# opteroncx/MoePhoto

Measured on AMD Instinct MI355X. Metric: megapixels/sec (input), 1080p 4x SR (Net4x a4), 256-px tiles with overlap, higher is better.
Workload: dtype fp16; 1 GPU; BASELINE configs[1]: 1 frame(s) 1920x1080 RGB -> 7680x4320, model a4 (Net4x, synthetic weights in zoo format), crop 256 pad 5 align 8 -> 40 tiles/frame, fp16 I/O, fp16 MFMA operands + fp32 accumulate; tiles_per_frame=40, parallelism=single GPU, precision=mixed, exact_blocks=1, input=natural-image-like synthetic frame (tests/golden_defs.natural_image)

## Files before the change

moephoto_amd/csrc/common.h:

```cpp
#pragma once
#include <hip/hip_runtime.h>
#include <stdint.h>

typedef _Float16 half_t;
typedef __attribute__((ext_vector_type(2))) _Float16 half2_t;
typedef __attribute__((ext_vector_type(4))) _Float16 half4_t;
typedef __attribute__((ext_vector_type(8))) _Float16 half8_t;
typedef __attribute__((ext_vector_type(4))) float float4_t;
typedef __attribute__((ext_vector_type(16))) float float16_t;

constexpr int kCB = 64;
constexpr int kTileW = 32;
constexpr int kTileH = 8;
constexpr int kFragBytes = 1024;

struct ConvArgs {
    const half_t* in;
    half_t* out;
    const half_t* res;
    const half_t* wpk;
    const float* bias;
    const float* bias_img;
    const half_t* zero;
    half_t* trash;
// ... 103 lines not shown
    const half_t* tail_w;
    half_t* out;
    float* plane;
    float* apron;
    float slope;
    int B, H, W;
    int split;
};
bool launch_conv3x3_ps4(const Ps4Args& a, int max_groups, hipStream_t s);
bool ps4_applicable(int B, int H, int W);
inline bool ps4_tail_applicable(int B, int H, int W, float slope) { return slope < 1.f && ps4_applicable(B, H, W); }
bool ps4_store_applicable(int B, int H, int W, float slope);
size_t ps4_plane_bytes(int B, int H, int W);
size_t ps4_apron_bytes(int B, int H, int W);
hipError_t conv3x3_ps4_init();
struct TailAddArgs {
    const float* p0; const float* p1;
    const float* a0; const float* a1;
    void* y; int y_dtype; const long long* y_off;
    int B, H, W, px;
    int vec_ok;
};
void launch_tailadd(const TailAddArgs& a, hipStream_t s);

struct Ps9Args {
    const half_t* in;
    const half_t* wpk;
    const float* bias;
    const half_t* tail_w;
    float* plane;
    float* apron;
    float slope;
    int B, H, W;
    int split;
    int xcd_map;
};
// ... 198 lines not shown
};
void launch_frm_pre(const FrmPreArgs& a, hipStream_t s);

struct StitchArgs {
    const float* tiles; const long long* tile_off;
    const int* row_first; const int* row_cnt;
    const int* col_first; const int* col_cnt;
    const int* row_tab; const int* col_tab;
    const float* ramp;
    void* out; int out_dtype;
    int C, out_h, out_w, step_w;
    int row_lo;
    int y0, rows;
};
void launch_stitch(const StitchArgs& a, hipStream_t s);

struct BlendTileArgs {
    const void* r; void* canvas; const void* ramp;
    long long r_sC, r_sH, c_sC, c_sH;
    int C, rh, rw;
    int top_sc, left_sc;
    int r0, c0;
    int lt_h, lt_w;
};
void launch_blend_tile(const BlendTileArgs& a, bool f16, hipStream_t s);

struct WireRec {
    long long tile_off, wire_off;
    int C, th, tw;
    int ra0, ra1, rb0, rb1;
// ... 12 lines not shown
```

moephoto_amd/csrc/conv3x3_ps4.hip:

```cpp
#include "common.h"
#include "rowtile.h"
#include "../../include/moephoto_amd.h"
#include <algorithm>
#include <type_traits>

#ifndef PS4_FILL
#define PS4_FILL 5
#endif
#ifndef PS4_ZSKIP
#define PS4_ZSKIP 1
#endif
#ifndef PS4_ABL
#define PS4_ABL 0
#endif

namespace {

constexpr int RB = 4;
constexpr int PW = kTileW + 2;
constexpr int ROWB = PW * 128;
constexpr int BLKB = RB * ROWB;
constexpr int NPIECE = BLKB / 1024;
constexpr int TREC = 36 * 128 + 64;
constexpr int TEXP = 36 * 128;
// ... 456 lines not shown
        typedef std::integral_constant<int, 0> Run;
        typedef std::integral_constant<int, 1> Zero;
        typedef std::integral_constant<int, 2> Last;
        int k = kfirst;
        for (; k + 1 < kz; k += 2) {
            block(k, std::integral_constant<int, 0>{}, Run{});
            block(k + 1, std::integral_constant<int, 1>{}, Run{});
        }
        if (k < kz) { block(k, std::integral_constant<int, 0>{}, Run{}); ++k; }
        if (k < nblk - 1) { block(k, std::integral_constant<int, 0>{}, Zero{}); ++k; }
        if (TAIL) block(k, std::integral_constant<int, 0>{}, Last{});
    }
#endif
}

template <bool VEC>
__global__ __launch_bounds__(256) void tailadd_kernel(TailAddArgs a)
{
    const int nq = a.W >> 3;
    const long long idx = (long long)blockIdx.x * 256 + threadIdx.x;
    if (idx >= (long long)a.B * a.H * nq) return;
    const int xq = (int)(idx % nq);
    const int Y = (int)((idx / nq) % a.H), b = (int)(idx / ((long long)nq * a.H));
    const int X0 = xq * 8;
    const long long po = ((long long)b * a.H + Y) * a.W + X0;
    float v[8];
    {
        const float4 r0 = *(const float4*)(a.p0 + po), r1 = *(const float4*)(a.p0 + po + 4);
        v[0] = r0.x; v[1] = r0.y; v[2] = r0.z; v[3] = r0.w; v[4] = r1.x; v[5] = r1.y; v[6] = r1.z; v[7] = r1.w;
        if (a.p1) {
            const float4 u0 = *(const float4*)(a.p1 + po), u1 = *(const float4*)(a.p1 + po + 4);
            v[0] += u0.x; v[1] += u0.y; v[2] += u0.z; v[3] += u0.w; v[4] += u1.x; v[5] += u1.y; v[6] += u1.z; v[7] += u1.w;
        }
    }
    const int c = X0 >> 6, in = X0 & 63;
    const long long as = (long long)a.B * a.px * a.H;
    if (in == 0 && c >= 1) {
        const long long o = ((long long)b * a.px + (c - 1)) * a.H + Y;
        float t = a.a0[o];
        if (a.a1) t += a.a1[o];
        v[0] += t;
    }
    if (in == 56 && c + 1 < a.px) {
        const long long o = as + ((long long)b * a.px + (c + 1)) * a.H + Y;
        float t = a.a0[o];
        if (a.a1) t += a.a1[o];
        v[7] += t;
    }
    const long long yo = (a.y_off ? a.y_off[b] : (long long)b * a.H * a.W) + (long long)Y * a.W + X0;
    if (a.y_dtype == MOE_F16) {
        if (VEC) {
            half8_t h;
#pragma unroll
            for (int k = 0; k < 8; ++k) h[k] = (half_t)v[k];
            *(half8_t*)((half_t*)a.y + yo) = h;
        } else {
#pragma unroll
            for (int k = 0; k < 8; ++k) ((half_t*)a.y)[yo + k] = (half_t)v[k];
        }
    } else {
        float* yp = (float*)a.y + yo;
        if (VEC) {
            *(float4*)yp = make_float4(v[0], v[1], v[2], v[3]);
            *(float4*)(yp + 4) = make_float4(v[4], v[5], v[6], v[7]);
        } else {
#pragma unroll
            for (int k = 0; k < 8; ++k) yp[k] = v[k];
        }
    }
}

template <int EPI, bool MASK>
hipError_t set_limit()
{
    return hipFuncSetAttribute((const void*)conv3x3_ps4_kernel<EPI, MASK>, hipFuncAttributeMaxDynamicSharedMemorySize, LDS_BYTES);
}

}

hipError_t conv3x3_ps4_init()
{
    hipError_t e;
    if ((e = set_limit<0, true>()) != hipSuccess) return e;
    if ((e = set_limit<1, false>()) != hipSuccess) return e;
// ... 49 lines not shown
```

moephoto_amd/csrc/engine.h:

```cpp
#pragma once
#include <cstdint>
#include <map>
#include <memory>
#include <string>
#include <utility>
#include <vector>

#include "../../include/moephoto_amd.h"
#include "common.h"

namespace moe {

struct AxisAnchors {
    std::vector<int64_t> start, end, end_sc;
    int64_t clip = 0;
    int step = 1;
};
AxisAnchors get_anchors(int64_t s, int64_t ns, int64_t l, int pad, int align, int sc);

struct TileRect { int top, bottom, left, right, top_t, left_t, bsc, rsc; };

struct PlanDeviceCache {
    int device = -1;
    int C = 0;
    int64_t sC = 0, sH = 0, sW = 0;
    int shard_index = 0, shard_count = 1;
    bool y_mult8 = false;
    std::vector<int> group_first, group_count;
    void* blob = nullptr;
    long long* x_off = nullptr;
    long long* y_off = nullptr;
    long long* tile_off = nullptr;
    int *row_first = nullptr, *row_cnt = nullptr, *col_first = nullptr, *col_cnt = nullptr, *row_tab = nullptr, *col_tab = nullptr;
    float* ramp = nullptr;
    std::vector<std::pair<int, int*>> strip_tabs;
};

struct FramesDeviceCache {
    int device = -1, C = 0, n_frames = 0;
    int64_t sC = 0, sH = 0, sW = 0, frame_stride = 0;
    std::vector<long long> tile_dst;
    bool y_mult8 = false;
    std::vector<int> group_first, group_count;
    void* blob = nullptr;
    long long* x_off = nullptr;
    long long* y_off = nullptr;
};

struct CustomOffsets { int device; std::vector<long long> host; long long* dev; };
// ... 24 lines not shown
```

moephoto_amd/csrc/forward.cpp:

```cpp
#include "net.h"

using namespace moe;

namespace moe {

const char* kernel_name(ConvKernel k)
{
    static const char* const names[] = {"no kernel", "conv_direct", "conv1x1", "conv_mfma", "conv3x3_sp", "conv3x3_rw", "conv3x3_ps4 (store form)", "conv3x3_sp (hi + lo residual)",
                                        "conv_mfma (three products)", "conv64_x3", "conv64_q8", "conv64_sq", "conv3x3_sp (three launches)", "conv_mfma (fp32 side buffer)"};
    return names[(int)k];
}

static bool fast_layer(const moe_net& n, const ConvLayer& L) { return L.taps == 9 && L.nseg == 1 && !L.per_plane && n.opt.conv_impl == 2; }

ConvForm Fwd::form(const ConvLayer& L, int H, int W) const
{
    ConvForm c;
    c.B = B; c.H = H; c.W = W; c.in_cs = 64 * L.nseg; c.out_cs = L.r > 1 ? 64 : 64 * L.nchunks; c.r = L.r; c.nchunks = L.nchunks;
    c.py = (H + kTileH - 1) / kTileH;
    const long long items = (long long)B * ((W + kTileW - 1) / kTileW) * c.py;
    const int per_xcd = groups / 8;
    int G = per_xcd >= L.nchunks ? 8 * (per_xcd / L.nchunks) : groups / L.nchunks;
    if (G < 1) G = 1;
    if (G > items) G = (int)items;
// ... 371 lines not shown
    if ((io.x_dtype != MOE_F32 && io.x_dtype != MOE_F16) || (io.y_dtype != MOE_F32 && io.y_dtype != MOE_F16))
        return fail(MOE_EINVAL, "moe_net_forward: x/y dtype must be MOE_F32 or MOE_F16");
    const long long bmax = kSpRange / (sp_bytes_per_pixel(n) * (long long)h * w);
    if (bmax < 1)
        return fail(MOE_ENOMEM, "a %dx%d tile exceeds the convolution kernels' addressing range (%lld pixels per plane at most for this net): use a smaller cropsize",
                    h, w, kSpRange / sp_bytes_per_pixel(n));
    if (n.arch == MOE_ARCH_LITE && io.x_dtype == MOE_F16 && n.lut_state == 0 && n.opt.lite_lut) build_lite_lut(n, s, ctx);
    if (B <= bmax) return forward_dev_chunk(n, io, B, h, w, s, y_off_mult8, ctx);
    const size_t xe = io.x_dtype == MOE_F32 ? 4 : 2, ye = io.y_dtype == MOE_F32 ? 4 : 2;
    const long long yplane = (long long)h * n.scale * w * n.scale;
    for (int b0 = 0; b0 < B; b0 += (int)bmax) {
        const int cnt = (int)std::min<long long>(bmax, B - b0);
        FwdIO c = io;
        if (io.x_off) c.x_off += b0; else c.x = (const char*)io.x + (size_t)b0 * io.sB * xe;
        if (io.y_off) c.y_off += b0; else c.y = (char*)io.y + (size_t)b0 * yplane * ye;
        const bool al = y_off_mult8 && (io.y_off || ((size_t)b0 * yplane * ye) % 16 == 0);
        if (int rc = forward_dev_chunk(n, c, cnt, h, w, s, al, ctx)) return rc;
    }
    return MOE_OK;
}

static int forward_dev_chunk(moe_net& n, const FwdIO& io, int B, int h, int w, hipStream_t s, bool y_off_mult8, const FwdCtx& ctx)
{
    int cur = -1;
    HIP_TRY(hipGetDevice(&cur));
    if (cur != n.device) HIP_TRY(hipSetDevice(n.device));
    const size_t need = workspace_need(n, ctx, B, h, w);
    StreamSet& set = *ctx.set;
    if (need > set.ws_bytes) {
        if (set.ws) { HIP_TRY(hipStreamSynchronize(s)); HIP_TRY(hipFree(set.ws)); set.ws = nullptr; set.ws_bytes = 0; }
        hipError_t e = hipMalloc((void**)&set.ws, need);
        if (e != hipSuccess) { (void)hipGetLastError(); return fail(MOE_ENOMEM, "workspace of %zu bytes for %d planes of %dx%d does not fit", need, B, h, w); }
        set.ws_bytes = need;
    }
// ... 210 lines not shown
```

moephoto_amd/csrc/forward_arsb.cpp:

```cpp
#include "net.h"

using namespace moe;

namespace {

const ConvLayer* last_up(const moe_net& n, int br)
{
    const auto it = n.conv_index.find(std::string(br == 0 ? "convt_R1" : "u") + ".up" + std::to_string(n.stages - 1));
    return it == n.conv_index.end() ? nullptr : &n.convs[it->second];
}

bool can_fuse_tail(const moe_net& n, const Fwd& f)
{
    const int B = f.B, h = f.h, w = f.w;
    if (!n.opt.fuse_tail || f.x3 || f.direct || n.debug || n.opt.conv_impl != 2 || n.stages < 1) return false;
    if (!(n.arch == MOE_ARCH_NET2X || n.arch == MOE_ARCH_NET3X || n.arch == MOE_ARCH_NET4X)) return false;
    if (sp_bytes_per_pixel(n) * B * h * w > kSpRange) return false;
    int hl = h, wl = w;
    for (int st = 0; st + 1 < n.stages; ++st) { hl *= n.r; wl *= n.r; }
    for (int br = 0; br < 2; ++br) {
        const ConvLayer* L = last_up(n, br);
        if (!L) return false;
        ConvForm c = f.form(*L, hl, wl);
        c.tail = true;
// ... 39 lines not shown
        bool ok = fuse && n.opt.tail_form == 1;
        bool ps4_ok = true;
        bool ps9_ok = true;
        for (int br = 0; br < 2; ++br) {
            const ConvLayer* L = last_up(n, br);
            if (ok) {
                ConvForm c = f.form(*L, hl, wl);
                c.tail = true; c.tail_form = 1;
                ok = conv3x3_rw_applicable(c);
            }
            ps4_ok = ps4_ok && L && ps4_tail_applicable(B, hl, wl, L->slope);
            ps9_ok = ps9_ok && L && ps9_tail_applicable(B, hl, wl, L->slope);
        }
        f.tail_form = ok ? 1 : 0;
        ps4 = ok && n.opt.up_impl == 1 && ps4_ok && (2 * wl) % 8 == 0;
        ps9 = fuse && n.opt.up_impl == 1 && n.r == 3 && f.groups >= 3 && ps9_ok;
    }
}

template <typename Args, typename Launch>
int ArsbRun::ps_stage(int br, const std::string& key, const Act& cur, size_t plane_bytes, size_t apron_bytes, const char* name, Launch launch)
{
    ps_plane[br] = (float*)f.ar.take(plane_bytes + 4096);
    ps_apron[br] = (float*)f.ar.take(apron_bytes + 4096);
    if (!f.dry()) {
        const ConvLayer& L = n.convs[n.conv_index.at(key)];
        Args q{};
        q.in = cur.hi; q.wpk = f.blob<half_t>(L.w_hi); q.bias = L.has_bias ? f.blob<float>(L.bias) : f.small<float>("zero_bias");
        q.tail_w = f.small<half_t>(br == 0 ? "tail_r.frag" : "tail_u.frag");
        q.plane = ps_plane[br]; q.apron = ps_apron[br]; q.slope = L.slope; q.B = B; q.H = H; q.W = W;
// ... 120 lines not shown
        if (int rc = trunk_conv(k2, m, cur, &resid, ex)) return rc;
        f.tap("arsb" + std::to_string(i), cur, h, w, 64, n.C);
    }
    Bb = cur;
    return (int)MOE_OK;
}

template <typename Args, typename Launch>
void ArsbRun::tail_add(Launch launch)
{
    if (f.dry()) return;
    Args t{};
    t.p0 = ps_plane[0]; t.p1 = ps_plane[1]; t.a0 = ps_apron[0]; t.a1 = ps_apron[1];
    t.y = f.io.y; t.y_dtype = f.io.y_dtype; t.y_off = f.io.y_off; t.B = B; t.H = H; t.W = W; t.px = (W / n.r + kTileW - 1) / kTileW;
    t.vec_ok = f.y_vec;
    const int rec = f.prof_begin("tailadd", 0.0);
    f.gate();
    launch(t, f.s);
    f.prof_end(rec);
}

int ArsbRun::branch_sum()
{
    if (ps4) { tail_add<TailAddArgs>(launch_tailadd); return MOE_OK; }
    if (ps9) { tail_add<TailAdd3Args>(launch_tailadd3); return MOE_OK; }
    if (fuse) {
        if (!f.dry()) {
            TapSumArgs t{};
            t.t0 = tp[0]; t.t1 = tp[1]; t.y = f.io.y; t.y_dtype = f.io.y_dtype; t.y_off = f.io.y_off; t.B = B; t.H = H; t.W = W; t.r = n.r;
            t.form = f.tail_form;
            t.vec_ok = n.r == 2 && f.y_vec && W % 8 == 0;
            f.gate();
            launch_tapsum(t, f.s);
        }
        return MOE_OK;
    }
    f.tail(&fin[0], &fin[1], H, W, false);
    return MOE_OK;
// ... 79 lines not shown
```

moephoto_amd/csrc/misc_kernels.hip:

```cpp
#include "common.h"
#include <algorithm>
#include <cstdlib>
#include <cstring>
#include "../../include/moephoto_amd.h"

namespace {

__device__ __forceinline__ float prelu(float v, float slope) { return v >= 0.f ? v : v * slope; }

template <typename T>
__device__ __forceinline__ float ld1(const void* p, long long i) { return (float)((const T*)p)[i]; }

template <typename TIN, int TAPS>
__global__ __launch_bounds__(256) void stem_kernel(StemArgs a)
{
    __shared__ float w[TAPS * 64];
    for (int i = threadIdx.x; i < TAPS * 64; i += 256) w[i] = a.w[i];
    __syncthreads();
    if (a.out_lo8) asm volatile("s_setreg_imm32_b32 hwreg(HW_REG_MODE, 23, 1), 1\n\ts_nop 3" ::: "memory");
    constexpr int PX = 8;
    const int nq = (a.W + PX - 1) / PX;
    const long long idx = (long long)blockIdx.x * 256 + threadIdx.x;
    const long long q = idx >> 3;
    if (q >= (long long)a.B * a.H * nq) return;
// ... 1091 lines not shown
    }
    __syncthreads();
    const int total = s_nseam * 8 * R;
    for (int t = threadIdx.x; t < total; t += 256) {
        const int gidx = t / (8 * R), rem = t - gidx * 8 * R;
        const int r = rem >> 3, e = rem & 7;
        const int X = (blockIdx.x * 256 + s_seam[gidx]) * 8 + e, Y = Y0 + r;
        if (Y >= yend) continue;
        const float cur = stitch_pixel(a, X, Y, c);
        const long long o = ((long long)c * a.rows + (Y - a.y0)) * a.out_w + X;
        if (a.out_dtype == MOE_F16) ((half_t*)a.out)[o] = (half_t)cur;
        else ((float*)a.out)[o] = cur;
    }
}

template <typename TS, typename TD>
__global__ void to_float_kernel(const TS* src, TD* dst, int H, int W, int C, float d, bool divide)
{
    const long long idx = (long long)blockIdx.x * 256 + threadIdx.x;
    const long long n = (long long)H * W * C;
    if (idx >= n) return;
    const int c = (int)(idx % C);
    const long long p = idx / C;
    const float v = (float)src[idx];
    dst[(long long)c * H * W + p] = (TD)(divide ? v / d : v * d);
}

template <typename TS, typename TD>
__global__ void to_output_kernel(const TS* src, TD* dst, int H, int W, int C, float quant)
{
// ... 143 lines not shown
    const long long total = (long long)a.B * a.HW * 8;
    hipLaunchKernelGGL(frm_apply_kernel, dim3((unsigned)((total + 255) / 256)), dim3(256), 0, s, a);
}

void launch_frm_pre(const FrmPreArgs& a, hipStream_t s)
{
    hipLaunchKernelGGL(frm_pre_kernel, dim3(a.B), dim3(256), 0, s, a);
}

void launch_stitch(const StitchArgs& a, hipStream_t s)
{
    if (a.rows <= 0) return;
    if (a.out_w % 8 == 0 && a.step_w <= 64 && ((uintptr_t)a.out & 15) == 0) hipLaunchKernelGGL(stitch8r_kernel<4>, dim3((a.out_w / 8 + 255) / 256, (a.rows + 3) / 4, a.C), dim3(256), 0, s, a);
    else if (a.out_w % 4 == 0 && ((uintptr_t)a.out & 15) == 0) hipLaunchKernelGGL(stitch4_kernel, dim3((a.out_w / 4 + 255) / 256, a.rows, a.C), dim3(256), 0, s, a);
    else hipLaunchKernelGGL(stitch_kernel, dim3((a.out_w + 255) / 256, a.rows, a.C), dim3(256), 0, s, a);
}

__device__ __forceinline__ int wire_slot(int v, int a0, int a1, int b0, int b1)
{
    return (v >= a0 && v < a1) ? v - a0 : (v >= b0 && v < b1) ? (a1 - a0) + v - b0 : -1;
}

template <bool PACK>
__global__ __launch_bounds__(256) void wire_kernel(float* __restrict__ tiles, unsigned* __restrict__ wire, const WireRec* __restrict__ recs)
{
    const WireRec r = recs[blockIdx.y];
    const int nR = (r.ra1 - r.ra0) + (r.rb1 - r.rb0), nC = (r.ca1 - r.ca0) + (r.cb1 - r.cb0);
    const bool raw = nR >= r.th;
    const long long plane = (long long)r.th * r.tw, n = plane * r.C;
    float* t = tiles + r.tile_off;
// ... 185 lines not shown
```

moephoto_amd/csrc/net.h:

```cpp
#pragma once
#include "engine.h"

#include <algorithm>
#include <cmath>
#include <cstdarg>
#include <cstdio>
#include <cstdlib>
#include <cstring>

namespace moe {

int fail(int code, const char* fmt, ...);

#define HIP_TRY(expr)                                                                                    \
    do {                                                                                                 \
        hipError_t e_ = (expr);                                                                          \
        if (e_ != hipSuccess) return fail(e_ == hipErrorOutOfMemory ? MOE_ENOMEM : MOE_EHIP, "%s: %s", #expr, hipGetErrorString(e_)); \
    } while (0)

struct Param {
    std::string name;
    std::vector<int64_t> shape;
    std::vector<float> data;
    bool set = false;
// ... 49 lines not shown
    int k48 = 1;
    int s64 = 1;
    int branch_streams = 1;
    int branch_groups = 0;
    int exact_fuse = 1;
    int q8_impl = 1;
    int fuse_tail = 1;
    int sedn_fuse = 1;
    int pool_fuse = 1;
    int lite_lut = 1;
    int stem2 = 1;
    int frm_pre = 1;
    int overlap_calls = 1;
    int overlap_fork = 0;
    int overlap_groups = 0;
    int calib_log = 0;
    int auto_calibrate = 1;
    int exact_blocks_env = -1;
    int tiles_per_batch = 0;
    int max_groups = 0;
    int dbg = 0;
    std::string trace_key = "convt_R1.up1";
    bool arsb_trace = false;
    std::string repeat_key;
    int repeat_n = 1;


    bool set(const std::string& key, const char* v);
    void from_env();
};
// ... 51 lines not shown
        return it == index.end() ? nullptr : &params[it->second];
    }
    void add(const std::string& n, std::vector<int64_t> shape)
    {
        index[n] = (int)params.size();
        moe::Param p; p.name = n; p.shape = std::move(shape);
        params.push_back(std::move(p));
    }
};

namespace moe {

struct FwdIO {
    const void* x = nullptr; int x_dtype = MOE_F32; long long sB = 0, sH = 0, sW = 0; const long long* x_off = nullptr;
    void* y = nullptr; int y_dtype = MOE_F32; const long long* y_off = nullptr;
};

struct FwdCtx {
    StreamSet* set = nullptr;
    int groups = 0;
    bool fork = false;
    hipEvent_t gate_event = nullptr;
    float* lut_capture = nullptr;
};
inline FwdCtx own_ctx(const moe_net& n, StreamSet* set) { return FwdCtx{set, n.max_groups, n.opt.branch_streams != 0, nullptr, nullptr}; }

struct ConvExtra {
    const half_t* plane_w = nullptr;
    const half_t* plane_w_lo = nullptr;
    const half_t* tail_w = nullptr;
// ... 17 lines not shown
enum class ConvKernel {
    none, direct, conv1x1,
    mfma, sp, rw, ps4_store,
    sp_res_lo,
    mfma_x3,
    x3, q8, sq,
    sp_three, acc32,
};
struct ConvRoute {
    ConvKernel kernel = ConvKernel::none;
    ConvDone done;
    ConvForm form;
    ConvX3Form x3;
};
const char* kernel_name(ConvKernel k);

struct Fwd {
    const moe_net& n;
    const FwdCtx& ctx;
    NetRuntime* rt;
    hipStream_t s;
    int B, h, w;
    Arena ar;
    int groups;
    bool x3, direct;
    bool mixed = false;
    bool y_vec = false;
    float* acc32 = nullptr;
    size_t acc32_elems = 0;
    half_t* side16 = nullptr;
    bool dry() const { return ar.base == nullptr; }
    int rc = 0;
    bool skips_planned_work = false;
    int tail_form = 0;
    FwdIO io;

    Act act(long long pixels, int ch = 64, bool want_lo = false)
    {
        Act a;
        a.hi = (half_t*)ar.take((size_t)pixels * ch * 2 + 2048);
        if (x3 || want_lo) { a.lo = (half_t*)ar.take((size_t)pixels * ch * 2 + 2048); a.has_lo = true; }
        return a;
    }
    template <typename T> T* blob(size_t off) const { return (T*)(n.blob + off); }
    template <typename T> T* small(const std::string& k) const { return (T*)(n.blob + n.small.at(k)); }

    void tap(const std::string& name, const Act& a, int H, int W, int cs, int C)
    {
        if (!n.debug || dry()) return;
        auto& t = rt->taps[name];
        if (t.dev) { (void)hipFree(t.dev); t.dev = nullptr; }
        const size_t nel = (size_t)B * C * H * W;
        if (hipMalloc((void**)&t.dev, nel * 4) != hipSuccess) return;
        t.shape[0] = B; t.shape[1] = C; t.shape[2] = H; t.shape[3] = W;
        launch_nhwc_to_nchw_f32(a.hi, a.lo, t.dev, B, H, W, cs, C, s);
    }

    bool tail_split_for(const std::string& key) const
    {
        const int mode = n.opt.tail_split;
        return mode == 2 || (mode == 1 && key.compare(0, 8, "convt_R1") == 0);
    }

    int prof_begin(const std::string& key, double flops)
    {
        for (size_t i = 0; i < n.prof_keys.size(); ++i) {
            if (key.find(n.prof_keys[i]) == std::string::npos) continue;
            if (rt->prof_used == rt->prof_ev.size()) {
                NetRuntime::ProfRec r;
                if (hipEventCreate(&r.e0) != hipSuccess || hipEventCreate(&r.e1) != hipSuccess) return -1;
                rt->prof_ev.push_back(r);
            }
            NetRuntime::ProfRec& r = rt->prof_ev[rt->prof_used];
            r.key = (int)i; r.flops = flops;
            (void)hipEventRecord(r.e0, s);
            return (int)rt->prof_used++;
        }
        return -1;
    }
    void prof_end(int rec) { if (rec >= 0) (void)hipEventRecord(rt->prof_ev[rec].e1, s); }
    int repeats(const std::string& key) const { return (!n.opt.repeat_key.empty() && key.find(n.opt.repeat_key) != std::string::npos) ? n.opt.repeat_n : 1; }

    bool use_q8() const { return mixed && (n.opt.x3_impl == 2 || (n.opt.x3_impl == 0 && (n.scale > 1 || n.arch == MOE_ARCH_NETDN))); }
    bool q8_capable(const ConvLayer& L) const
    {
        ConvX3Form c;
        c.B = B; c.H = h; c.W = w; c.slope = L.slope; c.in8 = c.out8 = true;
        return n.opt.x3_fuse && n.opt.conv_impl == 2 && L.k == 3 && L.r == 1 && L.nchunks == 1 && L.nseg == 1 && !L.per_plane && L.wq_hi8 && L.w_arsb_lo && !L.has_bias && conv64_q8_applicable(c);
    }

    ConvDone conv(const std::string& key, const Act& in, const Act& out, const Act* res, int H, int W, const ConvExtra& extra = ConvExtra{});
    ConvRoute route(const std::string& key, const Act& in, const Act& out, const Act* res, int H, int W, const ConvExtra& extra = ConvExtra{}) const;
    ConvForm form(const ConvLayer& L, int H, int W) const;
    int launch(const ConvRoute& r, const std::string& key, const Act& in, const Act& out, const Act* res, const ConvExtra& extra);
    void stem(const Act& out, const Act* out2 = nullptr);
    void tail(const Act* r, const Act* u, int H, int W, bool skip);
    void gate();
};

int forward_arsb(const moe_net& n, Fwd& f);
int forward_sedn(const moe_net& n, Fwd& f);
int forward_lite(const moe_net& n, Fwd& f);

int exact_blocks_of(const moe_net& n);
int default_exact_blocks(int arch);
long long sp_bytes_per_pixel(const moe_net& n);
constexpr long long kSpRange = (1ll << 32) - (1ll << 16);
int forward_dev(moe_net& n, const FwdIO& io, int B, int h, int w, hipStream_t s, bool y_off_mult8, const FwdCtx& ctx);
void free_set(StreamSet& set);
void pipe_destroy(moe_net& n);
void free_records(NetRuntime& rt);
int build_device_weights(moe_net& n, int precision);
void drop_lut(moe_net& n);
bool calibratable(const moe_net& n);
int calibrate_blocks(moe_net& n, double target, hipStream_t s);
int calibrate_sedn(moe_net& n, double target, hipStream_t s, bool adopt);

}
```

moephoto_amd/csrc/options.cpp:

```cpp
#include "net.h"

using namespace moe;

namespace {

enum OptionKind {
    kFlag,
    kWords,
    kCount,
    kInt,
    kText,
    kRepeat,
};
struct OptionWord { const char* word; int value; };
struct OptionRow {
    const char* key;
    const char* env;
    OptionKind kind;
    int NetOptions::*num;
    std::string NetOptions::*text;
    OptionWord words[3];
};
constexpr OptionWord kOnOff[] = {{"0", 0}, {"off", 0}, {"1", 1}, {"on", 1}};

// ... 33 lines not shown
    {"repeat", nullptr, kRepeat},
};

bool word_value(const OptionWord* words, size_t n, const char* v, int& out)
{
    for (size_t i = 0; i < n; ++i)
        if (words[i].word && !strcmp(v, words[i].word)) { out = words[i].value; return true; }
    return false;
}

}

bool NetOptions::set(const std::string& key, const char* v)
{
    if (!v) return false;
    for (const OptionRow& r : kOptionTable) {
        if (key != r.key) continue;
        int t = 0;
        switch (r.kind) {
            case kFlag: if (!word_value(kOnOff, 4, v, t)) return false; break;
            case kWords: if (!word_value(r.words, 3, v, t)) return false; break;
            case kCount: if ((t = atoi(v)) < 0) return false; break;
            case kInt: t = atoi(v); break;
            case kText: this->*r.text = v; return true;
            case kRepeat: {
                const char* c = strrchr(v, ':');
                if (!c) {
                    if (*v && strcmp(v, "0")) return false;
                    repeat_key.clear(); repeat_n = 1;
                    return true;
// ... 4 lines not shown
                return true;
            }
        }
        this->*r.num = t;
        return true;
    }
    return false;
}

void NetOptions::from_env()
{
    for (const OptionRow& r : kOptionTable)
        if (const char* e = r.env ? getenv(r.env) : nullptr)
            if (!set(r.key, e)) fprintf(stderr, "moephoto_amd: %s=\"%s\" is not a value of option %s -- ignored\n", r.env, e, r.key);

    if (const char* e = getenv("MOE_EXACT_BLOCKS")) exact_blocks_env = atoi(e);
    arsb_trace = getenv("MOE_ARSB_TRACE") != nullptr;
}

extern "C" int moe_net_set_option(moe_net* n, const char* key, const char* value)
{
    if (!n || !key || !value) return fail(MOE_EINVAL, "moe_net_set_option: NULL argument");
    if (!n->opt.set(key, value)) return fail(MOE_EINVAL, "moe_net_set_option: unknown option or value \"%s\" = \"%s\"", key, value);
    drop_lut(*n);
    if (!strcmp(key, "max_groups") && n->finalized) n->max_groups = n->opt.max_groups > 0 ? n->opt.max_groups : conv_mfma_max_groups();
    return MOE_OK;
}
```

moephoto_amd/csrc/plan_run.cpp:

```cpp
#include "net.h"

using namespace moe;

static int plan_device_tables(const Plan& p, int device, int C, int64_t sC, int64_t sH, int64_t sW, int si, int scnt,
                              PlanDeviceCache** outp)
{
    if (scnt < 1) { scnt = 1; si = 0; }
    for (auto& up : p.dev) {
        PlanDeviceCache& d = *up;
        if (d.blob && d.device == device && d.C == C && d.sC == sC && d.sH == sH && d.sW == sW && d.shard_index == si && d.shard_count == scnt) {
            *outp = &d;
            return MOE_OK;
        }
    }
    if (p.dev.size() >= 16) {
        if (p.dev.front()->blob) (void)hipFree(p.dev.front()->blob);
        for (auto& e : p.dev.front()->strip_tabs) (void)hipFree(e.second);
        p.dev.erase(p.dev.begin());
    }
    p.dev.push_back(std::make_unique<PlanDeviceCache>());
    PlanDeviceCache& d = *p.dev.back();
    const size_t nt = p.tiles.size();
    std::vector<long long> xo, yo;
    int slot = 0;
    for (const auto& g : p.groups) {
        d.group_first.push_back(slot);
        int cnt = 0;
        for (int k : g.tiles) {
            if (k % scnt != si) continue;
            const TileRect& t = p.tiles[k];
            const long long plane = (long long)(g.th * p.sc) * (g.tw * p.sc);
            for (int c = 0; c < C; ++c) {
                xo.push_back((long long)c * sC + (long long)t.top * sH + (long long)t.left * sW);
                yo.push_back(p.tile_off[k] / p.C * C + (long long)c * plane);
            }
            ++slot; ++cnt;
        }
        d.group_count.push_back(cnt);
    }
    if (xo.empty()) { xo.push_back(0); yo.push_back(0); }
    d.y_mult8 = true;
    for (long long v : yo) d.y_mult8 = d.y_mult8 && (v % 8 == 0);
    std::vector<long long> toff(nt);
    for (size_t k = 0; k < nt; ++k) toff[k] = p.tile_off[k] / p.C * C;
    std::vector<char> host;
    auto put = [&](const void* src, size_t bytes) { const size_t a = (host.size() + 255) & ~(size_t)255; host.resize(a + bytes); memcpy(host.data() + a, src, bytes); return a; };
    const size_t o_x = put(xo.data(), xo.size() * 8), o_y = put(yo.data(), yo.size() * 8), o_t = put(toff.data(), toff.size() * 8);
    const size_t o_rf = put(p.row_first.data(), p.row_first.size() * 4), o_rc = put(p.row_cnt.data(), p.row_cnt.size() * 4);
    const size_t o_cf = put(p.col_first.data(), p.col_first.size() * 4), o_cc = put(p.col_cnt.data(), p.col_cnt.size() * 4);
    const size_t o_rt = put(p.row_tab.data(), p.row_tab.size() * 4), o_ct = put(p.col_tab.data(), p.col_tab.size() * 4);
    const float zero = 0.f;
    const size_t o_rp = put(p.ramp.empty() ? &zero : p.ramp.data(), std::max<size_t>(4, p.ramp.size() * 4));
    HIP_TRY(hipMalloc(&d.blob, host.size()));
    HIP_TRY(hipMemcpy(d.blob, host.data(), host.size(), hipMemcpyHostToDevice));
    char* b = (char*)d.blob;
    d.x_off = (long long*)(b + o_x); d.y_off = (long long*)(b + o_y); d.tile_off = (long long*)(b + o_t);
    d.row_first = (int*)(b + o_rf); d.row_cnt = (int*)(b + o_rc); d.col_first = (int*)(b + o_cf); d.col_cnt = (int*)(b + o_cc);
    d.row_tab = (int*)(b + o_rt); d.col_tab = (int*)(b + o_ct); d.ramp = (float*)(b + o_rp);
    d.device = device; d.C = C; d.sC = sC; d.sH = sH; d.sW = sW; d.shard_index = si; d.shard_count = scnt;
    *outp = &d;
    return MOE_OK;
}

static void fill_stitch(const Plan& p, const PlanDeviceCache& d, StitchArgs& a, const float* tiles, const long long* tile_off, int C, void* out, int out_dtype)
{
    a.tiles = tiles; a.tile_off = tile_off;
    a.row_first = d.row_first; a.row_cnt = d.row_cnt; a.col_first = d.col_first; a.col_cnt = d.col_cnt;
    a.row_tab = d.row_tab; a.col_tab = d.col_tab; a.ramp = d.ramp;
    a.out = out; a.out_dtype = out_dtype; a.C = C; a.out_h = p.out_h; a.out_w = p.out_w; a.step_w = p.aw.step;
    a.y0 = 0; a.rows = p.out_h; a.row_lo = 0;
}

struct moe_plan { Plan p; };
// ... 243 lines not shown
int moe_run_plan_ex(moe_net* n, const moe_plan* pl, const void* img, int img_dtype, int64_t sC, int64_t sH, int64_t sW,
                    void* out, int out_dtype, int max_tiles, float* pool, int shard_index, int shard_count, int do_stitch, void* stream)
{
    if (!n || !pl || !img || (do_stitch && !out)) return fail(MOE_EINVAL, "moe_run_plan: NULL argument");
    if (!n->finalized) return fail(MOE_ESTATE, "moe_run_plan: net is not finalized");
    const Plan& p = pl->p;
    if (p.sc != n->scale) return fail(MOE_EINVAL, "moe_run_plan: plan scale %d != net scale %d", p.sc, n->scale);
    if (shard_count < 1) { shard_count = 1; shard_index = 0; }
    if (shard_index < 0 || shard_index >= shard_count) return fail(MOE_EINVAL, "moe_run_plan: shard %d of %d", shard_index, shard_count);
    hipStream_t s = (hipStream_t)stream;
    HIP_TRY(hipSetDevice(n->device));
    const int C = p.C;
    PlanDeviceCache* d = nullptr;
    int rc = plan_device_tables(p, n->device, C, sC, sH, sW, shard_index, shard_count, &d);
    if (rc) return rc;
    if (!pool) {
        const size_t pool_need = p.pool_elems_per_plane_set;
        if (pool_need > p.pool_elems) {
            if (p.pool) { HIP_TRY(hipStreamSynchronize(s)); HIP_TRY(hipFree(p.pool)); p.pool = nullptr; p.pool_elems = 0; }
            if (hipMalloc((void**)&p.pool, pool_need * 4) != hipSuccess) { (void)hipGetLastError(); return fail(MOE_ENOMEM, "tile pool of %zu bytes does not fit", pool_need * 4); }
            p.pool_elems = pool_need;
        }
        pool = p.pool;
    }
    if (max_tiles <= 0) {
        max_tiles = n->opt.tiles_per_batch > 0 ? n->opt.tiles_per_batch : 32;
    }
    for (size_t gi = 0; gi < p.groups.size(); ++gi) {
        const auto& g = p.groups[gi];
        const int nt = d->group_count[gi];
        if (nt < 1) continue;
        const long long px = (long long)g.th * g.tw;
        const int per = (int)std::max<long long>(1, std::min<long long>(nt, (long long)max_tiles * 65536 / std::max<long long>(px, 1)));
        for (int t0 = 0; t0 < nt; t0 += per) {
            const int cnt = std::min(per, nt - t0);
            const long long slot = (long long)(d->group_first[gi] + t0) * C;
            rc = forward_dev(*n, FwdIO{img, img_dtype, 0, sH, sW, d->x_off + slot, pool, MOE_F32, d->y_off + slot}, cnt * C, g.th, g.tw, s, d->y_mult8, own_ctx(*n, &n->set));
            if (rc) return rc;
        }
    }
    if (do_stitch) {
        StitchArgs a{};
        fill_stitch(p, *d, a, pool, d->tile_off, C, out, out_dtype);
        launch_stitch(a, s);
        hipError_t e = hipGetLastError();
        if (e != hipSuccess) return fail(MOE_EHIP, "stitch launch failed: %s", hipGetErrorString(e));
    }
    return MOE_OK;
}

int moe_run_plan_tiles(moe_net* n, const moe_plan* pl, const void* imgs, int img_dtype, int64_t frame_stride,
                       int64_t sC, int64_t sH, int64_t sW, int n_frames, float* dst, const int64_t* tile_dst,
                       int max_tiles, void* stream)
{
    if (!n || !pl || !imgs || !dst || !tile_dst || n_frames < 1) return fail(MOE_EINVAL, "moe_run_plan_tiles: bad argument");
    if (!n->finalized) return fail(MOE_ESTATE, "moe_run_plan_tiles: net is not finalized");
// ... 126 lines not shown
```

Before: 87.63 MP/s.

## Write tile interiors straight to the output canvas from tailadd, stitch only seams

The final ps4 branch-sum kernel now writes each tile's solely-owned interior pixels directly into the output image. Only pixels that are not exclusively owned go to the fp32 tile pool. A seam-only stitch kernel then blends the overlap rows and columns, replacing the full-frame stitch pass that reread every tile pixel. This removes most of the stitch kernel's memory traffic at 4x output resolution, at the cost of per-pixel ownership branches in tailadd, an extra dry-run check of the forward path, and two small seam launches.

After: 88.16 MP/s, median of 6. About the same (+0.6%).

```diff
diff --git a/moephoto_amd/csrc/common.h b/moephoto_amd/csrc/common.h
--- a/moephoto_amd/csrc/common.h
+++ b/moephoto_amd/csrc/common.h
@@ -141,12 +141,19 @@
 size_t ps4_plane_bytes(int B, int H, int W);
 size_t ps4_apron_bytes(int B, int H, int W);
 hipError_t conv3x3_ps4_init();
+struct CanvasPlane {
+    long long base;
+    int oy, ox;
+    int ry0, ry1, rx0, rx1;
+    int ch, cw;
+};
 struct TailAddArgs {
     const float* p0; const float* p1;
     const float* a0; const float* a1;
     void* y; int y_dtype; const long long* y_off;
     int B, H, W, px;
     int vec_ok;
+    void* canvas; int canvas_dtype; const CanvasPlane* canvas_tab; int canvas_w; int canvas_vec;
 };
 void launch_tailadd(const TailAddArgs& a, hipStream_t s);
 
@@ -375,6 +382,7 @@
     int y0, rows;
 };
 void launch_stitch(const StitchArgs& a, hipStream_t s);
+void launch_stitch_seams(const StitchArgs& a, const int* rows, int nrows, const int* cols, int ncols, hipStream_t s);
 
 struct BlendTileArgs {
     const void* r; void* canvas; const void* ramp;
diff --git a/moephoto_amd/csrc/conv3x3_ps4.hip b/moephoto_amd/csrc/conv3x3_ps4.hip
--- a/moephoto_amd/csrc/conv3x3_ps4.hip
+++ b/moephoto_amd/csrc/conv3x3_ps4.hip
@@ -494,17 +494,9 @@
 #endif
 }
 
-template <bool VEC>
-__global__ __launch_bounds__(256) void tailadd_kernel(TailAddArgs a)
-{
-    const int nq = a.W >> 3;
-    const long long idx = (long long)blockIdx.x * 256 + threadIdx.x;
-    if (idx >= (long long)a.B * a.H * nq) return;
-    const int xq = (int)(idx % nq);
-    const int Y = (int)((idx / nq) % a.H), b = (int)(idx / ((long long)nq * a.H));
-    const int X0 = xq * 8;
+__device__ __forceinline__ void tailadd_sum(const TailAddArgs& a, int b, int Y, int X0, float (&v)[8])
+{
     const long long po = ((long long)b * a.H + Y) * a.W + X0;
-    float v[8];
     {
         const float4 r0 = *(const float4*)(a.p0 + po), r1 = *(const float4*)(a.p0 + po + 4);
         v[0] = r0.x; v[1] = r0.y; v[2] = r0.z; v[3] = r0.w; v[4] = r1.x; v[5] = r1.y; v[6] = r1.z; v[7] = r1.w;
@@ -527,6 +519,79 @@
         if (a.a1) t += a.a1[o];
         v[7] += t;
     }
+}
+
+__device__ __forceinline__ void tailadd_store_f32(float* yp, const float (&v)[8], bool vec)
+{
+    if (vec) {
+        *(float4*)yp = make_float4(v[0], v[1], v[2], v[3]);
+        *(float4*)(yp + 4) = make_float4(v[4], v[5], v[6], v[7]);
+    } else {
+#pragma unroll
+        for (int k = 0; k < 8; ++k) yp[k] = v[k];
+    }
+}
+
+template <bool VEC>
+__device__ __forceinline__ void tailadd_to_canvas(const TailAddArgs& a, int b, int Y, int X0)
+{
+    const CanvasPlane e = a.canvas_tab[b];
+    if (Y >= e.ch || X0 >= e.cw) return;
+    float v[8];
+    tailadd_sum(a, b, Y, X0, v);
+    const bool rowin = Y >= e.ry0 && Y < e.ry1;
+    const int lo = rowin ? max(e.rx0 - X0, 0) : 8, hi = rowin ? min(e.rx1 - X0, 8) : 0;
+    const int non = min(e.cw - X0, 8);
+    const long long yo = a.y_off[b] + (long long)Y * a.W + X0;
+    const long long co = e.base + (long long)(e.oy + Y) * a.canvas_w + e.ox + X0;
+    float* yp = (float*)a.y + yo;
+    if (lo == 0 && hi == 8) {
+        if (a.canvas_dtype == MOE_F16) {
+            half_t* cp = (half_t*)a.canvas + co;
+            if (a.canvas_vec && (co & 7) == 0) {
+                half8_t h;
+#pragma unroll
+                for (int k = 0; k < 8; ++k) h[k] = (half_t)v[k];
+                *(half8_t*)cp = h;
+            } else if (a.canvas_vec && (co & 3) == 0) {
+                half4_t h0, h1;
+#pragma unroll
+                for (int k = 0; k < 4; ++k) { h0[k] = (half_t)v[k]; h1[k] = (half_t)v[4 + k]; }
+                *(half4_t*)cp = h0;
+                *(half4_t*)(cp + 4) = h1;
+            } else {
+#pragma unroll
+                for (int k = 0; k < 8; ++k) cp[k] = (half_t)v[k];
+            }
+        } else
+            tailadd_store_f32((float*)a.canvas + co, v, a.canvas_vec && (co & 3) == 0);
+    } else if (lo >= hi && non == 8) {
+        tailadd_store_f32(yp, v, VEC);
+    } else {
+#pragma unroll
+        for (int k = 0; k < 8; ++k) {
+            if (k >= non) continue;
+            if (k >= lo && k < hi) {
+                if (a.canvas_dtype == MOE_F16) ((half_t*)a.canvas)[co + k] = (half_t)v[k];
+                else ((float*)a.canvas)[co + k] = v[k];
+            } else
+                yp[k] = v[k];
+        }
+    }
+}
+
+template <bool VEC>
+__global__ __launch_bounds__(256) void tailadd_kernel(TailAddArgs a)
+{
+    const int nq = a.W >> 3;
+    const long long idx = (long long)blockIdx.x * 256 + threadIdx.x;
+    if (idx >= (long long)a.B * a.H * nq) return;
+    const int xq = (int)(idx % nq);
+    const int Y = (int)((idx / nq) % a.H), b = (int)(idx / ((long long)nq * a.H));
+    const int X0 = xq * 8;
+    if (a.canvas) { tailadd_to_canvas<VEC>(a, b, Y, X0); return; }
+    float v[8];
+    tailadd_sum(a, b, Y, X0, v);
     const long long yo = (a.y_off ? a.y_off[b] : (long long)b * a.H * a.W) + (long long)Y * a.W + X0;
     if (a.y_dtype == MOE_F16) {
         if (VEC) {
@@ -538,16 +603,8 @@
 #pragma unroll
             for (int k = 0; k < 8; ++k) ((half_t*)a.y)[yo + k] = (half_t)v[k];
         }
-    } else {
-        float* yp = (float*)a.y + yo;
-        if (VEC) {
-            *(float4*)yp = make_float4(v[0], v[1], v[2], v[3]);
-            *(float4*)(yp + 4) = make_float4(v[4], v[5], v[6], v[7]);
-        } else {
-#pragma unroll
-            for (int k = 0; k < 8; ++k) yp[k] = v[k];
-        }
-    }
+    } else
+        tailadd_store_f32((float*)a.y + yo, v, VEC);
 }
 
 template <int EPI, bool MASK>
diff --git a/moephoto_amd/csrc/engine.h b/moephoto_amd/csrc/engine.h
--- a/moephoto_amd/csrc/engine.h
+++ b/moephoto_amd/csrc/engine.h
@@ -33,6 +33,10 @@
     long long* tile_off = nullptr;
     int *row_first = nullptr, *row_cnt = nullptr, *col_first = nullptr, *col_cnt = nullptr, *row_tab = nullptr, *col_tab = nullptr;
     float* ramp = nullptr;
+    bool canvas_ok = false;
+    CanvasPlane* canvas_tab = nullptr;
+    int *seam_rows = nullptr, *own_rows = nullptr, *seam_cols = nullptr;
+    int n_seam_rows = 0, n_own_rows = 0, n_seam_cols = 0;
     std::vector<std::pair<int, int*>> strip_tabs;
 };
 
diff --git a/moephoto_amd/csrc/forward.cpp b/moephoto_amd/csrc/forward.cpp
--- a/moephoto_amd/csrc/forward.cpp
+++ b/moephoto_amd/csrc/forward.cpp
@@ -409,10 +409,23 @@
         FwdIO c = io;
         if (io.x_off) c.x_off += b0; else c.x = (const char*)io.x + (size_t)b0 * io.sB * xe;
         if (io.y_off) c.y_off += b0; else c.y = (char*)io.y + (size_t)b0 * yplane * ye;
+        if (io.canvas_tab) c.canvas_tab += b0;
         const bool al = y_off_mult8 && (io.y_off || ((size_t)b0 * yplane * ye) % 16 == 0);
         if (int rc = forward_dev_chunk(n, c, cnt, h, w, s, al, ctx)) return rc;
     }
     return MOE_OK;
+}
+
+bool forward_sum_is_ps4(const moe_net& n, const FwdCtx& ctx, int B, int h, int w)
+{
+    if (!n.finalized || B < 1 || h < 1 || w < 1) return false;
+    const long long bmax = kSpRange / (sp_bytes_per_pixel(n) * (long long)h * w);
+    if (bmax < 1) return false;
+    for (int b0 = 0; b0 < B; b0 += (int)std::min<long long>(bmax, B)) {
+        Fwd f = make_fwd(n, ctx, nullptr, nullptr, (int)std::min<long long>(bmax, B - b0), h, w, Arena{});
+        if (run_forward(n, f, FwdIO{}) != MOE_OK || !f.sum_ps4) return false;
+    }
+    return true;
 }
 
 static int forward_dev_chunk(moe_net& n, const FwdIO& io, int B, int h, int w, hipStream_t s, bool y_off_mult8, const FwdCtx& ctx)
diff --git a/moephoto_amd/csrc/forward_arsb.cpp b/moephoto_amd/csrc/forward_arsb.cpp
--- a/moephoto_amd/csrc/forward_arsb.cpp
+++ b/moephoto_amd/csrc/forward_arsb.cpp
@@ -1,4 +1,6 @@
 #include "net.h"
+
+#include <type_traits>
 
 using namespace moe;
 
@@ -77,6 +79,7 @@
         }
         f.tail_form = ok ? 1 : 0;
         ps4 = ok && n.opt.up_impl == 1 && ps4_ok && (2 * wl) % 8 == 0;
+        f.sum_ps4 = ps4;
         ps9 = fuse && n.opt.up_impl == 1 && n.r == 3 && f.groups >= 3 && ps9_ok;
     }
 }
@@ -227,7 +230,15 @@
     t.p0 = ps_plane[0]; t.p1 = ps_plane[1]; t.a0 = ps_apron[0]; t.a1 = ps_apron[1];
     t.y = f.io.y; t.y_dtype = f.io.y_dtype; t.y_off = f.io.y_off; t.B = B; t.H = H; t.W = W; t.px = (W / n.r + kTileW - 1) / kTileW;
     t.vec_ok = f.y_vec;
-    const int rec = f.prof_begin("tailadd", 0.0);
+    const char* key = "tailadd";
+    if constexpr (std::is_same<Args, TailAddArgs>::value) {
+        if (f.io.canvas) {
+            t.canvas = f.io.canvas; t.canvas_dtype = f.io.canvas_dtype; t.canvas_tab = f.io.canvas_tab; t.canvas_w = f.io.canvas_w;
+            t.canvas_vec = ((uintptr_t)f.io.canvas & 15) == 0;
+            key = "tailadd_canvas";
+        }
+    }
+    const int rec = f.prof_begin(key, 0.0);
     f.gate();
     launch(t, f.s);
     f.prof_end(rec);
@@ -235,6 +246,8 @@
 
 int ArsbRun::branch_sum()
 {
+    if (f.io.canvas && !(ps4 && f.io.y_off && f.io.y_dtype == MOE_F32))
+        return fail(MOE_EINVAL, "internal error: a forward was handed the canvas, and its branch sum is not the ps4 form into an fp32 pool");
     if (ps4) { tail_add<TailAddArgs>(launch_tailadd); return MOE_OK; }
     if (ps9) { tail_add<TailAdd3Args>(launch_tailadd3); return MOE_OK; }
     if (fuse) {
diff --git a/moephoto_amd/csrc/misc_kernels.hip b/moephoto_amd/csrc/misc_kernels.hip
--- a/moephoto_amd/csrc/misc_kernels.hip
+++ b/moephoto_amd/csrc/misc_kernels.hip
@@ -1129,6 +1129,18 @@
     }
 }
 
+__global__ __launch_bounds__(256) void stitch_seam_kernel(StitchArgs a, const int* rows, int nrows, const int* cols, int ncols)
+{
+    const long long idx = (long long)blockIdx.x * 256 + threadIdx.x;
+    if (idx >= (long long)nrows * ncols) return;
+    const int k = (int)(idx % ncols), l = (int)(idx / ncols), c = blockIdx.y;
+    const int X = cols ? cols[k] : k, Y = rows[l];
+    const float cur = stitch_pixel(a, X, Y, c);
+    const long long o = ((long long)c * a.out_h + Y) * a.out_w + X;
+    if (a.out_dtype == MOE_F16) ((half_t*)a.out)[o] = (half_t)cur;
+    else ((float*)a.out)[o] = cur;
+}
+
 template <typename TS, typename TD>
 __global__ void to_float_kernel(const TS* src, TD* dst, int H, int W, int C, float d, bool divide)
 {
@@ -1302,6 +1314,13 @@
     if (a.out_w % 8 == 0 && a.step_w <= 64 && ((uintptr_t)a.out & 15) == 0) hipLaunchKernelGGL(stitch8r_kernel<4>, dim3((a.out_w / 8 + 255) / 256, (a.rows + 3) / 4, a.C), dim3(256), 0, s, a);
     else if (a.out_w % 4 == 0 && ((uintptr_t)a.out & 15) == 0) hipLaunchKernelGGL(stitch4_kernel, dim3((a.out_w / 4 + 255) / 256, a.rows, a.C), dim3(256), 0, s, a);
     else hipLaunchKernelGGL(stitch_kernel, dim3((a.out_w + 255) / 256, a.rows, a.C), dim3(256), 0, s, a);
+}
+
+void launch_stitch_seams(const StitchArgs& a, const int* rows, int nrows, const int* cols, int ncols, hipStream_t s)
+{
+    if (nrows < 1 || ncols < 1) return;
+    const long long n = (long long)nrows * ncols;
+    hipLaunchKernelGGL(stitch_seam_kernel, dim3((unsigned)((n + 255) / 256), a.C), dim3(256), 0, s, a, rows, nrows, cols, ncols);
 }
 
 __device__ __forceinline__ int wire_slot(int v, int a0, int a1, int b0, int b1)
diff --git a/moephoto_amd/csrc/net.h b/moephoto_amd/csrc/net.h
--- a/moephoto_amd/csrc/net.h
+++ b/moephoto_amd/csrc/net.h
@@ -87,6 +87,7 @@
     int overlap_calls = 1;
     int overlap_fork = 0;
     int overlap_groups = 0;
+    int direct_canvas = 1;
     int calib_log = 0;
     int auto_calibrate = 1;
     int exact_blocks_env = -1;
@@ -168,6 +169,7 @@
 struct FwdIO {
     const void* x = nullptr; int x_dtype = MOE_F32; long long sB = 0, sH = 0, sW = 0; const long long* x_off = nullptr;
     void* y = nullptr; int y_dtype = MOE_F32; const long long* y_off = nullptr;
+    void* canvas = nullptr; int canvas_dtype = MOE_F32; const CanvasPlane* canvas_tab = nullptr; int canvas_w = 0;
 };
 
 struct FwdCtx {
@@ -215,6 +217,24 @@
     ConvX3Form x3;
 };
 const char* kernel_name(ConvKernel k);
+
+inline int prof_begin(const moe_net& n, NetRuntime& rt, hipStream_t s, const std::string& key, double flops)
+{
+    for (size_t i = 0; i < n.prof_keys.size(); ++i) {
+        if (key.find(n.prof_keys[i]) == std::string::npos) continue;
+        if (rt.prof_used == rt.prof_ev.size()) {
+            NetRuntime::ProfRec r;
+            if (hipEventCreate(&r.e0) != hipSuccess || hipEventCreate(&r.e1) != hipSuccess) return -1;
+            rt.prof_ev.push_back(r);
+        }
+        NetRuntime::ProfRec& r = rt.prof_ev[rt.prof_used];
+        r.key = (int)i; r.flops = flops;
+        (void)hipEventRecord(r.e0, s);
+        return (int)rt.prof_used++;
+    }
+    return -1;
+}
+inline void prof_end(NetRuntime& rt, hipStream_t s, int rec) { if (rec >= 0) (void)hipEventRecord(rt.prof_ev[rec].e1, s); }
 
 struct Fwd {
     const moe_net& n;
@@ -233,6 +253,7 @@
     bool dry() const { return ar.base == nullptr; }
     int rc = 0;
     bool skips_planned_work = false;
+    bool sum_ps4 = false;
     int tail_form = 0;
     FwdIO io;
 
@@ -263,23 +284,8 @@
         return mode == 2 || (mode == 1 && key.compare(0, 8, "convt_R1") == 0);
     }
 
-    int prof_begin(const std::string& key, double flops)
-    {
-        for (size_t i = 0; i < n.prof_keys.size(); ++i) {
-            if (key.find(n.prof_keys[i]) == std::string::npos) continue;
-            if (rt->prof_used == rt->prof_ev.size()) {
-                NetRuntime::ProfRec r;
-                if (hipEventCreate(&r.e0) != hipSuccess || hipEventCreate(&r.e1) != hipSuccess) return -1;
-                rt->prof_ev.push_back(r);
-            }
-            NetRuntime::ProfRec& r = rt->prof_ev[rt->prof_used];
-            r.key = (int)i; r.flops = flops;
-            (void)hipEventRecord(r.e0, s);
-            return (int)rt->prof_used++;
-        }
-        return -1;
-    }
-    void prof_end(int rec) { if (rec >= 0) (void)hipEventRecord(rt->prof_ev[rec].e1, s); }
+    int prof_begin(const std::string& key, double flops) { return moe::prof_begin(n, *rt, s, key, flops); }
+    void prof_end(int rec) { moe::prof_end(*rt, s, rec); }
     int repeats(const std::string& key) const { return (!n.opt.repeat_key.empty() && key.find(n.opt.repeat_key) != std::string::npos) ? n.opt.repeat_n : 1; }
 
     bool use_q8() const { return mixed && (n.opt.x3_impl == 2 || (n.opt.x3_impl == 0 && (n.scale > 1 || n.arch == MOE_ARCH_NETDN))); }
@@ -308,6 +314,7 @@
 long long sp_bytes_per_pixel(const moe_net& n);
 constexpr long long kSpRange = (1ll << 32) - (1ll << 16);
 int forward_dev(moe_net& n, const FwdIO& io, int B, int h, int w, hipStream_t s, bool y_off_mult8, const FwdCtx& ctx);
+bool forward_sum_is_ps4(const moe_net& n, const FwdCtx& ctx, int B, int h, int w);
 void free_set(StreamSet& set);
 void pipe_destroy(moe_net& n);
 void free_records(NetRuntime& rt);
diff --git a/moephoto_amd/csrc/options.cpp b/moephoto_amd/csrc/options.cpp
--- a/moephoto_amd/csrc/options.cpp
+++ b/moephoto_amd/csrc/options.cpp
@@ -71,6 +71,12 @@
 bool NetOptions::set(const std::string& key, const char* v)
 {
     if (!v) return false;
+    if (key == "direct_canvas") {
+        int t = 0;
+        if (!word_value(kOnOff, 4, v, t)) return false;
+        direct_canvas = t;
+        return true;
+    }
     for (const OptionRow& r : kOptionTable) {
         if (key != r.key) continue;
         int t = 0;
@@ -105,6 +111,8 @@
         if (const char* e = r.env ? getenv(r.env) : nullptr)
             if (!set(r.key, e)) fprintf(stderr, "moephoto_amd: %s=\"%s\" is not a value of option %s -- ignored\n", r.env, e, r.key);
 
+    if (const char* e = getenv("MOE_DIRECT_CANVAS"))
+        if (!set("direct_canvas", e)) fprintf(stderr, "moephoto_amd: MOE_DIRECT_CANVAS=\"%s\" is not a value of option direct_canvas -- ignored\n", e);
     if (const char* e = getenv("MOE_EXACT_BLOCKS")) exact_blocks_env = atoi(e);
     arsb_trace = getenv("MOE_ARSB_TRACE") != nullptr;
 }
diff --git a/moephoto_amd/csrc/plan_run.cpp b/moephoto_amd/csrc/plan_run.cpp
--- a/moephoto_amd/csrc/plan_run.cpp
+++ b/moephoto_amd/csrc/plan_run.cpp
@@ -1,6 +1,23 @@
 #include "net.h"
 
 using namespace moe;
+
+static bool axis_owners(const std::vector<int>& tab, int out_len, std::vector<std::pair<int, int>>& own, std::vector<int>& seams, std::vector<int>& others)
+{
+    const int n = (int)tab.size() / 4;
+    own.assign((size_t)n, {0, 0});
+    std::vector<char> owned((size_t)out_len, 0);
+    for (int i = 0; i < n; ++i) {
+        const int first = tab[i * 4 + 0], solid = tab[i * 4 + 1], origin = tab[i * 4 + 2], end = std::min(origin + tab[i * 4 + 3], out_len);
+        if (first < origin || solid < first || (i + 1 < n && tab[(i + 1) * 4 + 0] < first)) return false;
+        const int hi = std::min(i + 1 < n ? tab[(i + 1) * 4 + 0] : out_len, end);
+        own[(size_t)i] = {std::min(solid, hi), hi};
+        for (int v = own[(size_t)i].first; v < hi; ++v) owned[(size_t)v] = 1;
+    }
+    seams.clear(); others.clear();
+    for (int v = 0; v < out_len; ++v) (owned[(size_t)v] ? others : seams).push_back(v);
+    return true;
+}
 
 static int plan_device_tables(const Plan& p, int device, int C, int64_t sC, int64_t sH, int64_t sW, int si, int scnt,
                               PlanDeviceCache** outp)
@@ -22,6 +39,10 @@
     PlanDeviceCache& d = *p.dev.back();
     const size_t nt = p.tiles.size();
     std::vector<long long> xo, yo;
+    std::vector<CanvasPlane> cv;
+    std::vector<std::pair<int, int>> own_r, own_c;
+    std::vector<int> seam_rows, own_rows, seam_cols, own_cols;
+    d.canvas_ok = axis_owners(p.row_tab, p.out_h, own_r, seam_rows, own_rows) && axis_owners(p.col_tab, p.out_w, own_c, seam_cols, own_cols);
     int slot = 0;
     for (const auto& g : p.groups) {
         d.group_first.push_back(slot);
@@ -30,15 +51,20 @@
             if (k % scnt != si) continue;
             const TileRect& t = p.tiles[k];
             const long long plane = (long long)(g.th * p.sc) * (g.tw * p.sc);
+            const int i = k / p.aw.step, j = k % p.aw.step;
             for (int c = 0; c < C; ++c) {
                 xo.push_back((long long)c * sC + (long long)t.top * sH + (long long)t.left * sW);
                 yo.push_back(p.tile_off[k] / p.C * C + (long long)c * plane);
+                if (!d.canvas_ok) continue;
+                const int oy = p.row_tab[i * 4 + 2], ox = p.col_tab[j * 4 + 2];
+                cv.push_back(CanvasPlane{(long long)c * p.out_h * p.out_w, oy, ox, own_r[(size_t)i].first - oy, own_r[(size_t)i].second - oy, own_c[(size_t)j].first - ox, own_c[(size_t)j].second - ox,
+                                         std::min(p.row_tab[i * 4 + 3], p.out_h - oy), std::min(p.col_tab[j * 4 + 3], p.out_w - ox)});
             }
             ++slot; ++cnt;
         }
         d.group_count.push_back(cnt);
     }
-    if (xo.empty()) { xo.push_back(0); yo.push_back(0); }
+    if (xo.empty()) { xo.push_back(0); yo.push_back(0); d.canvas_ok = false; }
     d.y_mult8 = true;
     for (long long v : yo) d.y_mult8 = d.y_mult8 && (v % 8 == 0);
     std::vector<long long> toff(nt);
@@ -51,12 +77,18 @@
     const size_t o_rt = put(p.row_tab.data(), p.row_tab.size() * 4), o_ct = put(p.col_tab.data(), p.col_tab.size() * 4);
     const float zero = 0.f;
     const size_t o_rp = put(p.ramp.empty() ? &zero : p.ramp.data(), std::max<size_t>(4, p.ramp.size() * 4));
+    const int none = 0;
+    auto put_ints = [&](const std::vector<int>& v) { return put(v.empty() ? &none : v.data(), std::max<size_t>(4, v.size() * 4)); };
+    const size_t o_cv = put(cv.empty() ? (const void*)&none : (const void*)cv.data(), std::max<size_t>(4, cv.size() * sizeof(CanvasPlane)));
+    const size_t o_sr = put_ints(seam_rows), o_or = put_ints(own_rows), o_sc = put_ints(seam_cols);
     HIP_TRY(hipMalloc(&d.blob, host.size()));
     HIP_TRY(hipMemcpy(d.blob, host.data(), host.size(), hipMemcpyHostToDevice));
     char* b = (char*)d.blob;
     d.x_off = (long long*)(b + o_x); d.y_off = (long long*)(b + o_y); d.tile_off = (long long*)(b + o_t);
     d.row_first = (int*)(b + o_rf); d.row_cnt = (int*)(b + o_rc); d.col_first = (int*)(b + o_cf); d.col_cnt = (int*)(b + o_cc);
     d.row_tab = (int*)(b + o_rt); d.col_tab = (int*)(b + o_ct); d.ramp = (float*)(b + o_rp);
+    d.canvas_tab = (CanvasPlane*)(b + o_cv); d.seam_rows = (int*)(b + o_sr); d.own_rows = (int*)(b + o_or); d.seam_cols = (int*)(b + o_sc);
+    d.n_seam_rows = (int)seam_rows.size(); d.n_own_rows = (int)own_rows.size(); d.n_seam_cols = (int)seam_cols.size();
     d.device = device; d.C = C; d.sC = sC; d.sH = sH; d.sW = sW; d.shard_index = si; d.shard_count = scnt;
     *outp = &d;
     return MOE_OK;
@@ -330,6 +362,7 @@
     PlanDeviceCache* d = nullptr;
     int rc = plan_device_tables(p, n->device, C, sC, sH, sW, shard_index, shard_count, &d);
     if (rc) return rc;
+    const bool own_pool = !pool;
     if (!pool) {
         const size_t pool_need = p.pool_elems_per_plane_set;
         if (pool_need > p.pool_elems) {
@@ -342,20 +375,41 @@
     if (max_tiles <= 0) {
         max_tiles = n->opt.tiles_per_batch > 0 ? n->opt.tiles_per_batch : 32;
     }
+    struct LaunchSet { long long slot; int planes, th, tw; };
+    std::vector<LaunchSet> sets;
     for (size_t gi = 0; gi < p.groups.size(); ++gi) {
         const auto& g = p.groups[gi];
         const int nt = d->group_count[gi];
         if (nt < 1) continue;
         const long long px = (long long)g.th * g.tw;
         const int per = (int)std::max<long long>(1, std::min<long long>(nt, (long long)max_tiles * 65536 / std::max<long long>(px, 1)));
-        for (int t0 = 0; t0 < nt; t0 += per) {
-            const int cnt = std::min(per, nt - t0);
-            const long long slot = (long long)(d->group_first[gi] + t0) * C;
-            rc = forward_dev(*n, FwdIO{img, img_dtype, 0, sH, sW, d->x_off + slot, pool, MOE_F32, d->y_off + slot}, cnt * C, g.th, g.tw, s, d->y_mult8, own_ctx(*n, &n->set));
-            if (rc) return rc;
-        }
-    }
-    if (do_stitch) {
+        for (int t0 = 0; t0 < nt; t0 += per) sets.push_back({(long long)(d->group_first[gi] + t0) * C, std::min(per, nt - t0) * C, g.th, g.tw});
+    }
+    const FwdCtx ctx = own_ctx(*n, &n->set);
+    bool direct = own_pool && do_stitch && shard_count == 1 && n->opt.direct_canvas && d->canvas_ok && (out_dtype == MOE_F16 || out_dtype == MOE_F32) && !sets.empty();
+    for (size_t k = 0; direct && k < sets.size(); ++k) {
+        bool seen = false;
+        for (size_t q = 0; q < k; ++q) seen = seen || (sets[q].planes == sets[k].planes && sets[q].th == sets[k].th && sets[q].tw == sets[k].tw);
+        direct = seen || forward_sum_is_ps4(*n, ctx, sets[k].planes, sets[k].th, sets[k].tw);
+    }
+    for (const LaunchSet& ls : sets) {
+        FwdIO io{img, img_dtype, 0, sH, sW, d->x_off + ls.slot, pool, MOE_F32, d->y_off + ls.slot};
+        if (direct) { io.canvas = out; io.canvas_dtype = out_dtype; io.canvas_tab = d->canvas_tab + ls.slot; io.canvas_w = p.out_w; }
+        rc = forward_dev(*n, io, ls.planes, ls.th, ls.tw, s, d->y_mult8, ctx);
+        if (rc) return rc;
+    }
+    if (direct) {
+        StitchArgs a{};
+        fill_stitch(p, *d, a, pool, d->tile_off, C, out, out_dtype);
+        if (d->n_seam_rows > 0 || d->n_seam_cols > 0) {
+            const int rec = prof_begin(*n, n->rt, s, "seam_fold", 0.0);
+            launch_stitch_seams(a, d->seam_rows, d->n_seam_rows, nullptr, p.out_w, s);
+            launch_stitch_seams(a, d->own_rows, d->n_own_rows, d->seam_cols, d->n_seam_cols, s);
+            prof_end(n->rt, s, rec);
+        }
+        hipError_t e = hipGetLastError();
+        if (e != hipSuccess) return fail(MOE_EHIP, "seam fold launch failed: %s", hipGetErrorString(e));
+    } else if (do_stitch) {
         StitchArgs a{};
         fill_stitch(p, *d, a, pool, d->tile_off, C, out, out_dtype);
         launch_stitch(a, s);
```
